# zju3dv/SMAP

Hardware: NVIDIA H100
Metric: end-to-end FPS @832x512 (backbone+association+lift) (higher is better)
Workload: dtype bf16x3 (split-bf16 operands, fp32 accumulate; fp32-faithful)

## Files before the change

smap_b200/csrc/conv_tc.cuh:

```cuda
#pragma once
#include <cuda.h>
#include "common.cuh"

namespace smapb {

struct alignas(64) ConvParams {
    CUtensorMap tmA;
    CUtensorMap tmA2;
    CUtensorMap tmB;
    CUtensorMap tmO;
    CUtensorMap tmR[3];
    int Hout, Wout, Nimg;
    int tw_log2, th;
    int tiles_x, tiles_y;
    int Cout;
    int kh, kw, stride, pad_y, pad_x;
    int kchunks;
    int kchunks2, stride2;
    int n_tiles;
    int total_tiles;
    const float* bias;
    int has_res;
    int n_post;
    __nv_bfloat16* out;
    float* out_f32;
    long long plane_stride;
    int relu;
    int reverse;
    int up_mode, up_Hi, up_Wi, up_pw, up_ph;
    long long* dbg;
    long long* dbg_tl;
    unsigned long long* sat;
};

__device__ __forceinline__ void tma_load_5d(uint32_t dst, const CUtensorMap* map, uint64_t* bar, int c0, int c1,
                                            int c2, int c3, int c4) {
    asm volatile(
        "cp.async.bulk.tensor.5d.shared::cluster.global.tile.mbarrier::complete_tx::bytes [%0], [%1, {%3, %4, %5, %6, "
        "%7}], [%2];" ::"r"(dst),
        "l"(map), "r"(smem_u32(bar)), "r"(c0), "r"(c1), "r"(c2), "r"(c3), "r"(c4)
        : "memory");
}
__device__ __forceinline__ void tma_load_4d(uint32_t dst, const CUtensorMap* map, uint64_t* bar, int c0, int c1,
                                            int c2, int c3) {
    asm volatile(
        "cp.async.bulk.tensor.4d.shared::cluster.global.tile.mbarrier::complete_tx::bytes [%0], [%1, {%3, %4, %5, "
        "%6}], [%2];" ::"r"(dst),
        "l"(map), "r"(smem_u32(bar)), "r"(c0), "r"(c1), "r"(c2), "r"(c3)
        : "memory");
}
__device__ __forceinline__ void tma_prefetch_desc(const CUtensorMap* map) {
    asm volatile("prefetch.tensormap [%0];" ::"l"(map) : "memory");
}
__device__ __forceinline__ void tma_store_5d(const CUtensorMap* map, uint32_t src, int c0, int c1, int c2, int c3,
                                             int c4) {
    asm volatile("cp.async.bulk.tensor.5d.global.shared::cta.tile.bulk_group [%0, {%2, %3, %4, %5, %6}], [%1];" ::"l"(map),
                 "r"(src), "r"(c0), "r"(c1), "r"(c2), "r"(c3), "r"(c4)
                 : "memory");
}
__device__ __forceinline__ void bulk_commit() { asm volatile("cp.async.bulk.commit_group;" ::: "memory"); }
template <int N>
__device__ __forceinline__ void bulk_wait_read() {
    asm volatile("cp.async.bulk.wait_group.read %0;" ::"n"(N) : "memory");
}
__device__ __forceinline__ void bulk_wait_all() { asm volatile("cp.async.bulk.wait_group 0;" ::: "memory"); }
enum { TURN_MAIN = 3, TURN_RING = 5 };
__device__ __forceinline__ void epi_bar_sync(int wg) { asm volatile("bar.sync %0, 128;" ::"r"(1 + wg) : "memory"); }
__device__ __forceinline__ void turn_wait(int turn, int wg) { asm volatile("bar.sync %0, 256;" ::"r"(turn + wg) : "memory"); }
__device__ __forceinline__ void turn_pass(int turn, int wg) { asm volatile("bar.arrive %0, 256;" ::"r"(turn + wg) : "memory"); }
template <int R>
__device__ __forceinline__ void setmaxnreg_dec() {
    asm volatile("setmaxnreg.dec.sync.aligned.u32 %0;" ::"n"(R));
}
template <int R>
__device__ __forceinline__ void setmaxnreg_inc() {
    asm volatile("setmaxnreg.inc.sync.aligned.u32 %0;" ::"n"(R));
}
struct ConvDbg {
    enum {
        PRODUCER_WAIT_EMPTY = 0,
        TOTAL = 1,
        CTAS = 2,
        CONS = 3,
        WAIT_FULL = 0,
        WAIT_ORDER = 1,
        EPILOGUE = 2,
        WAIT_RING = 3,
        WAIT_STAGE = 4,
        CONS_N = 5,
        COUNT = CONS + 2 * CONS_N
    };
};
__device__ __forceinline__ uint32_t lds_u32(uint32_t addr) {
    uint32_t r;
    asm volatile("ld.shared.u32 %0, [%1];" : "=r"(r) : "r"(addr));
    return r;
}
__device__ __forceinline__ void sts_u32(uint32_t addr, uint32_t v) {
    asm volatile("st.shared.u32 [%0], %1;" ::"r"(addr), "r"(v) : "memory");
}
__device__ __forceinline__ uint32_t sw64_off(int r, int j) { return (uint32_t)(r * 64 + ((j ^ ((r >> 1) & 3)) << 4)); }

__device__ __forceinline__ float up_scale(int in, int out) { return out > 1 ? (float)(in - 1) / (float)(out - 1) : 0.f; }
__device__ __forceinline__ int up_src_index(int dst, int in, int out) { return (int)(up_scale(in, out) * (float)dst); }

__device__ __forceinline__ float2 planes_to_f2(uint32_t h, uint32_t l) {
    return make_float2(bf16lo_to_f(h) + bf16lo_to_f(l), bf16hi_to_f(h) + bf16hi_to_f(l));
}

__device__ __forceinline__ uint64_t wgmma_desc_sw128(uint32_t smem_addr) {
    uint64_t d = 0;
    d |= (uint64_t)((smem_addr >> 4) & 0x3FFF);
    d |= (uint64_t)1 << 16;
    d |= (uint64_t)(1024 >> 4) << 32;
    d |= (uint64_t)1 << 62;
    return d;
}
__device__ __forceinline__ void wgmma_fence() { asm volatile("wgmma.fence.sync.aligned;" ::: "memory"); }
__device__ __forceinline__ void wgmma_commit() { asm volatile("wgmma.commit_group.sync.aligned;" ::: "memory"); }
template <int N>
__device__ __forceinline__ void wgmma_wait() {
    asm volatile("wgmma.wait_group.sync.aligned %0;" ::"n"(N) : "memory");
}
template <class E>
__device__ __forceinline__ void wgmma_m64n128(float (&d)[64], uint64_t adesc, uint64_t bdesc, uint32_t accumulate) {
#define SMAPB_WGMMA(TY) \
    asm volatile( \
        "{\n\t.reg .pred p;\n\tsetp.ne.b32 p, %66, 0;\n\t" \
        "wgmma.mma_async.sync.aligned.m64n128k16.f32." TY "." TY " {%0, %1, %2, %3, %4, %5, %6, %7, %8, %9, %10, %11, %12, " \
        "%13, %14, %15, %16, %17, %18, %19, %20, %21, %22, %23, %24, %25, %26, %27, %28, %29, %30, %31, %32, %33, %34, %35, " \
        "%36, %37, %38, %39, %40, %41, %42, %43, %44, %45, %46, %47, %48, %49, %50, %51, %52, %53, %54, %55, %56, %57, %58, " \
        "%59, %60, %61, %62, %63}, %64, %65, p, 1, 1, 0, 0;\n\t}" \
        : "+f"(d[0]), "+f"(d[1]), "+f"(d[2]), "+f"(d[3]), "+f"(d[4]), "+f"(d[5]), "+f"(d[6]), "+f"(d[7]), "+f"(d[8]), \
          "+f"(d[9]), "+f"(d[10]), "+f"(d[11]), "+f"(d[12]), "+f"(d[13]), "+f"(d[14]), "+f"(d[15]), "+f"(d[16]), \
          "+f"(d[17]), "+f"(d[18]), "+f"(d[19]), "+f"(d[20]), "+f"(d[21]), "+f"(d[22]), "+f"(d[23]), "+f"(d[24]), \
          "+f"(d[25]), "+f"(d[26]), "+f"(d[27]), "+f"(d[28]), "+f"(d[29]), "+f"(d[30]), "+f"(d[31]), "+f"(d[32]), \
          "+f"(d[33]), "+f"(d[34]), "+f"(d[35]), "+f"(d[36]), "+f"(d[37]), "+f"(d[38]), "+f"(d[39]), "+f"(d[40]), \
          "+f"(d[41]), "+f"(d[42]), "+f"(d[43]), "+f"(d[44]), "+f"(d[45]), "+f"(d[46]), "+f"(d[47]), "+f"(d[48]), \
          "+f"(d[49]), "+f"(d[50]), "+f"(d[51]), "+f"(d[52]), "+f"(d[53]), "+f"(d[54]), "+f"(d[55]), "+f"(d[56]), \
          "+f"(d[57]), "+f"(d[58]), "+f"(d[59]), "+f"(d[60]), "+f"(d[61]), "+f"(d[62]), "+f"(d[63]) \
        : "l"(adesc), "l"(bdesc), "r"(accumulate))
    if constexpr (E::F16) SMAPB_WGMMA("f16");
    else SMAPB_WGMMA("bf16");
#undef SMAPB_WGMMA
}
template <class E>
__device__ __forceinline__ void wgmma_m64n64(float (&d)[32], uint64_t adesc, uint64_t bdesc, uint32_t accumulate) {
#define SMAPB_WGMMA(TY) \
    asm volatile( \
        "{\n\t.reg .pred p;\n\tsetp.ne.b32 p, %34, 0;\n\t" \
        "wgmma.mma_async.sync.aligned.m64n64k16.f32." TY "." TY " {%0, %1, %2, %3, %4, %5, %6, %7, %8, %9, %10, %11, %12, " \
        "%13, %14, %15, %16, %17, %18, %19, %20, %21, %22, %23, %24, %25, %26, %27, %28, %29, %30, %31}, %32, %33, p, 1, " \
        "1, 0, 0;\n\t}" \
        : "+f"(d[0]), "+f"(d[1]), "+f"(d[2]), "+f"(d[3]), "+f"(d[4]), "+f"(d[5]), "+f"(d[6]), "+f"(d[7]), "+f"(d[8]), \
          "+f"(d[9]), "+f"(d[10]), "+f"(d[11]), "+f"(d[12]), "+f"(d[13]), "+f"(d[14]), "+f"(d[15]), "+f"(d[16]), \
          "+f"(d[17]), "+f"(d[18]), "+f"(d[19]), "+f"(d[20]), "+f"(d[21]), "+f"(d[22]), "+f"(d[23]), "+f"(d[24]), \
          "+f"(d[25]), "+f"(d[26]), "+f"(d[27]), "+f"(d[28]), "+f"(d[29]), "+f"(d[30]), "+f"(d[31]) \
        : "l"(adesc), "l"(bdesc), "r"(accumulate))
    if constexpr (E::F16) SMAPB_WGMMA("f16");
    else SMAPB_WGMMA("bf16");
#undef SMAPB_WGMMA
}
template <class E>
__device__ __forceinline__ void wgmma_m64n32(float (&d)[16], uint64_t adesc, uint64_t bdesc, uint32_t accumulate) {
#define SMAPB_WGMMA(TY) \
    asm volatile( \
        "{\n\t.reg .pred p;\n\tsetp.ne.b32 p, %18, 0;\n\t" \
        "wgmma.mma_async.sync.aligned.m64n32k16.f32." TY "." TY " {%0, %1, %2, %3, %4, %5, %6, %7, %8, %9, %10, %11, %12, " \
        "%13, %14, %15}, %16, %17, p, 1, 1, 0, 0;\n\t}" \
        : "+f"(d[0]), "+f"(d[1]), "+f"(d[2]), "+f"(d[3]), "+f"(d[4]), "+f"(d[5]), "+f"(d[6]), "+f"(d[7]), "+f"(d[8]), \
          "+f"(d[9]), "+f"(d[10]), "+f"(d[11]), "+f"(d[12]), "+f"(d[13]), "+f"(d[14]), "+f"(d[15]) \
        : "l"(adesc), "l"(bdesc), "r"(accumulate))
    if constexpr (E::F16) SMAPB_WGMMA("f16");
    else SMAPB_WGMMA("bf16");
#undef SMAPB_WGMMA
}
template <int BLOCK_N, class E>
__device__ __forceinline__ void wgmma_tile(float (&d)[BLOCK_N / 2], uint64_t adesc, uint64_t bdesc, uint32_t accumulate) {
    if constexpr (BLOCK_N == 128) wgmma_m64n128<E>(d, adesc, bdesc, accumulate);
    else if constexpr (BLOCK_N == 64) wgmma_m64n64<E>(d, adesc, bdesc, accumulate);
    else wgmma_m64n32<E>(d, adesc, bdesc, accumulate);
}

__device__ __forceinline__ long long mbar_wait_timed(uint64_t* bar, uint32_t parity, bool timed) {
    if (!timed) {
        mbar_wait(bar, parity);
        return 0;
    }
    const long long t0 = clock64();
    mbar_wait(bar, parity);
    return clock64() - t0;
}

template <int BLOCK_N, int NTERMS, int RING>
struct ConvCfg {
    static constexpr int TA = (NTERMS == 3) ? 2 : 1;
    static constexpr int A_BYTES = 128 * 128;
    static constexpr int B_BYTES = BLOCK_N * 128;
    static constexpr int STAGE_BYTES = TA * (A_BYTES + B_BYTES);
    static constexpr int CHUNKS = BLOCK_N / 32;
    static constexpr int CHUNK_BYTES = 128 * 64;
    static constexpr int SLOT_BYTES = TA * CHUNK_BYTES;
    static constexpr int RES_BUFS = RING ? 2 : 0;
    static constexpr int RES_DIV = RING ? RES_BUFS : 1;
    static constexpr int SMEM_LIMIT = 227 * 1024;
    static constexpr int stages_with(int out_bufs) {
        return (SMEM_LIMIT - 2048 - (out_bufs + RES_BUFS) * SLOT_BYTES) / STAGE_BYTES > 8
                   ? 8
                   : (SMEM_LIMIT - 2048 - (out_bufs + RES_BUFS) * SLOT_BYTES) / STAGE_BYTES;
    }
    static constexpr int OUT_PER_WG = stages_with(4) == stages_with(2) ? 2 : 1;
    static constexpr int OUT_BUFS = 2 * OUT_PER_WG;
    static constexpr int EPI_BYTES = (OUT_BUFS + RES_BUFS) * SLOT_BYTES;
    static constexpr int STAGES = stages_with(OUT_BUFS);
    static constexpr int SMEM_BYTES = STAGES * STAGE_BYTES + EPI_BYTES + 2048;
    static_assert(STAGES >= 2, "need at least a double buffer");
    static_assert(BLOCK_N == 32 || BLOCK_N == 64 || BLOCK_N == 128, "BLOCK_N");
};

template <int BLOCK_N, int NTERMS, int RING, class E>
__global__ void __launch_bounds__(384, 1) conv_tc_kernel(const __grid_constant__ ConvParams p) {
    static_assert(!E::F16 || NTERMS == 1, "fp16 operands are single-term");
    using Cfg = ConvCfg<BLOCK_N, NTERMS, RING>;
    constexpr int STAGES = Cfg::STAGES;
    constexpr bool UP = (RING == 2);
    extern __shared__ unsigned char smem_raw[];
    uint64_t* full_bar = reinterpret_cast<uint64_t*>(smem_raw);
    uint64_t* empty_bar = full_bar + STAGES;
    uint64_t* rfull_bar = empty_bar + STAGES;
    uint64_t* rempty_bar = rfull_bar + Cfg::RES_BUFS;
    const uint32_t ring = (smem_u32(smem_raw) + 1024u + 1023u) & ~1023u;
    const uint32_t out_stage = ring + STAGES * Cfg::STAGE_BYTES;
    const uint32_t res_stage = out_stage + Cfg::OUT_BUFS * Cfg::SLOT_BYTES;

    const int warp = threadIdx.x >> 5;
    const int lane = threadIdx.x & 31;
    const bool tl = p.dbg_tl != nullptr && blockIdx.x == 0;
    if (tl && threadIdx.x == 0) p.dbg_tl[0] = clock64();
    const int n_extra = RING ? p.has_res + p.n_post : 0;
    const bool tma_out = p.out != nullptr;

    if (warp == 0 && lane == 0) {
        tma_prefetch_desc(&p.tmA);
        tma_prefetch_desc(&p.tmB);
        if (p.kchunks2) tma_prefetch_desc(&p.tmA2);
        if (tma_out) tma_prefetch_desc(&p.tmO);
        for (int e = 0; e < n_extra; e++) tma_prefetch_desc(&p.tmR[e]);
    }
    if (warp == 1 && lane == 0) {
        for (int s = 0; s < STAGES; s++) {
            mbar_init(&full_bar[s], 1);
            mbar_init(&empty_bar[s], 4);
        }
        for (int s = 0; s < Cfg::RES_BUFS; s++) {
            mbar_init(&rfull_bar[s], 1);
            mbar_init(&rempty_bar[s], 128);
        }
        fence_mbar_init();
    }
    __syncthreads();

    const int num_kb1 = p.kh * p.kw * p.kchunks;
    const int num_kb = num_kb1 + p.kchunks2;
    const int tiles_per_img = p.tiles_x * p.tiles_y;
    const int tw = 1 << p.tw_log2;

    if (tl && threadIdx.x == 0) p.dbg_tl[1] = clock64();
    pdl_wait();
    pdl_trigger();
    const long long t_begin = p.dbg ? clock64() : 0;

    if (warp < 4) {
        setmaxnreg_dec<40>();
        if (warp == 0 && lane == 0) {
            int stage = 0;
            uint32_t phase = 0;
            long long w_empty = 0;
            for (int tile = blockIdx.x; tile < p.total_tiles; tile += gridDim.x) {
                const int te = p.reverse ? p.total_tiles - 1 - tile : tile;
                const int nt = te % p.n_tiles, mt = te / p.n_tiles;
                const int img = mt / tiles_per_img, r = mt - img * tiles_per_img;
                const int ty = r / p.tiles_x, tx = r - ty * p.tiles_x;
                const int x_in0 = (tx << p.tw_log2) * p.stride - p.pad_x;
                const int y_in0 = ty * p.th * p.stride - p.pad_y;
                for (int kb = 0; kb < num_kb; kb++) {
                    w_empty += mbar_wait_timed(&empty_bar[stage], phase ^ 1u, p.dbg != nullptr);
                    const uint32_t sbase = ring + stage * Cfg::STAGE_BYTES;
                    mbar_arrive_expect_tx(&full_bar[stage], Cfg::STAGE_BYTES);
                    const int brow = nt * BLOCK_N;
                    int kcol, tapc, ax, ay;
                    const CUtensorMap* amap;
                    if (kb < num_kb1) {
                        const int ts = kb / p.kchunks, kc = kb - ts * p.kchunks;
                        const int kx = ts / p.kh, ky = ts - kx * p.kh;
                        amap = &p.tmA, kcol = kc * 64, tapc = ky * p.kw + kx, ax = x_in0 + kx, ay = y_in0 + ky;
                    } else {
                        const int kc2 = kb - num_kb1;
                        amap = &p.tmA2, kcol = kc2 * 64, tapc = 0;
                        ax = (tx << p.tw_log2) * p.stride2, ay = ty * p.th * p.stride2;
                    }
                    const int wcol = (kb < num_kb1) ? kcol : (p.kchunks * 64 + kcol);
#pragma unroll
                    for (int t = 0; t < Cfg::TA; t++) {
                        const uint32_t da = sbase + t * Cfg::A_BYTES, db = sbase + Cfg::TA * Cfg::A_BYTES + t * Cfg::B_BYTES;
                        tma_load_5d(da, amap, &full_bar[stage], kcol, ax, ay, img, t);
                        tma_load_4d(db, &p.tmB, &full_bar[stage], wcol, brow, tapc, t);
                    }
                    if (++stage == STAGES) {
                        stage = 0;
                        phase ^= 1u;
                    }
                }
            }
            if (p.dbg) atomicAdd((unsigned long long*)&p.dbg[ConvDbg::PRODUCER_WAIT_EMPTY], (unsigned long long)w_empty);
        } else if (warp == 1 && lane == 0 && n_extra > 0) {
            int cnt = 0;
            for (int tile = blockIdx.x; tile < p.total_tiles; tile += gridDim.x) {
                const int te = p.reverse ? p.total_tiles - 1 - tile : tile;
                const int nt = te % p.n_tiles, mt = te / p.n_tiles;
                const int img = mt / tiles_per_img, r = mt - img * tiles_per_img;
                const int ty = r / p.tiles_x, tx = r - ty * p.tiles_x;
                for (int c = 0; c < Cfg::CHUNKS; c++) {
                    for (int e = 0; e < n_extra; e++) {
                        const int m = cnt++;
                        const int slot = m % Cfg::RES_DIV;
                        mbar_wait(&rempty_bar[slot], ((uint32_t)(m / Cfg::RES_DIV) & 1u) ^ 1u);
                        int cx = tx << p.tw_log2, cy = ty * p.th;
                        uint32_t bytes = Cfg::SLOT_BYTES;
                        if (UP && e == 0) {
                            cx = up_src_index(cx, p.up_Wi, p.Wout);
                            cy = up_src_index(cy, p.up_Hi, p.Hout);
                            bytes = (uint32_t)(p.up_pw * p.up_ph * 64 * Cfg::TA);
                        }
                        mbar_arrive_expect_tx(&rfull_bar[slot], bytes);
#pragma unroll
                        for (int t = 0; t < Cfg::TA; t++)
                            tma_load_5d(res_stage + slot * Cfg::SLOT_BYTES + t * Cfg::CHUNK_BYTES, &p.tmR[e],
                                        &rfull_bar[slot], nt * BLOCK_N + c * 32, cx, cy, img, t);
                    }
                }
            }
        }
    } else {
        setmaxnreg_inc<232>();
        const int wg = (warp >> 2) - 1;
        const int q4 = lane & 3;
        const int rw = (warp & 3) * 16 + (lane >> 2);
        const bool leader = (threadIdx.x & 127) == 0;
        const bool timed = p.dbg != nullptr && leader;
        const uint32_t ob0 = out_stage + (uint32_t)(wg * Cfg::OUT_PER_WG) * Cfg::SLOT_BYTES;
        const int n_cta = (p.total_tiles - (int)blockIdx.x + (int)gridDim.x - 1) / (int)gridDim.x;
        long long* const dc = p.dbg ? p.dbg + ConvDbg::CONS + ConvDbg::CONS_N * wg : nullptr;
        auto tally = [&](int k, long long cycles) {
            if (timed) atomicAdd((unsigned long long*)&dc[k], (unsigned long long)cycles);
        };
        float acc[2][BLOCK_N / 2];
        for (int j = wg; j < n_cta; j += 2) {
            const int tile = blockIdx.x + j * gridDim.x;
            const int te = p.reverse ? p.total_tiles - 1 - tile : tile;
            const int nt = te % p.n_tiles, mt = te / p.n_tiles;
            const int img = mt / tiles_per_img, r = mt - img * tiles_per_img;
            const int ty = r / p.tiles_x, tx = r - ty * p.tiles_x;
            const int n0 = nt * BLOCK_N;

            const uint32_t it0 = (uint32_t)j * (uint32_t)num_kb;
            int stage = (int)(it0 % STAGES);
            uint32_t phase = (it0 / STAGES) & 1u;
            if (j > 0) {
                const long long t0 = timed ? clock64() : 0;
                turn_wait(TURN_MAIN, wg);
                tally(ConvDbg::WAIT_ORDER, timed ? clock64() - t0 : 0);
            }
            int prev_stage = -1;
            uint32_t w_full = 0;
            for (int kb = 0; kb < num_kb; kb++) {
                w_full += (uint32_t)mbar_wait_timed(&full_bar[stage], phase, timed);
                if (tl && leader && j == 0 && kb == 0) p.dbg_tl[2] = clock64();
                const uint32_t sbase = ring + stage * Cfg::STAGE_BYTES;
                const uint64_t a0 = wgmma_desc_sw128(sbase);
                const uint64_t b0 = wgmma_desc_sw128(sbase + Cfg::TA * Cfg::A_BYTES);
                constexpr uint64_t A_STEP = (uint64_t)(Cfg::A_BYTES >> 4), B_STEP = (uint64_t)(Cfg::B_BYTES >> 4);
                constexpr uint64_t A_HALF = (uint64_t)((64 * 128) >> 4);
                wgmma_fence();
#pragma unroll
                for (int k = 0; k < 4; k++) {
#pragma unroll
                    for (int h = 0; h < 2; h++) {
                        const uint64_t ka = a0 + (uint64_t)(k * 2) + h * A_HALF, kbd = b0 + (uint64_t)(k * 2);
                        wgmma_tile<BLOCK_N, E>(acc[h], ka, kbd, (kb | k) != 0);
                        if (NTERMS == 3) {
                            wgmma_tile<BLOCK_N, E>(acc[h], ka + A_STEP, kbd, 1u);
                            wgmma_tile<BLOCK_N, E>(acc[h], ka, kbd + B_STEP, 1u);
                        }
                    }
                }
                wgmma_commit();
                wgmma_wait<1>();
                if (prev_stage >= 0 && lane == 0) mbar_arrive(&empty_bar[prev_stage]);
                prev_stage = stage;
                if (++stage == STAGES) {
                    stage = 0;
                    phase ^= 1u;
                }
            }
            if (j + 1 < n_cta) turn_pass(TURN_MAIN, wg ^ 1);
            tally(ConvDbg::WAIT_FULL, w_full);
            wgmma_wait<0>();
            if (lane == 0) mbar_arrive(&empty_bar[prev_stage]);
            if (tl && leader && j == n_cta - 1) p.dbg_tl[3] = clock64();

            const long long t_epi0 = timed ? clock64() : 0;
            int py[4], px[4];
            bool valid[4];
            long long pix[4];
#pragma unroll
            for (int q = 0; q < 4; q++) {
                const int row = 64 * (q >> 1) + rw + 8 * (q & 1);
                py[q] = ty * p.th + (row >> p.tw_log2);
                px[q] = (tx << p.tw_log2) + (row & (tw - 1));
                valid[q] = (py[q] < p.Hout) && (px[q] < p.Wout) && (img < p.Nimg);
                pix[q] = ((long long)img * p.Hout + py[q]) * p.Wout + px[q];
            }
            auto row_of = [&](int q) { return 64 * (q >> 1) + rw + 8 * (q & 1); };
            const bool ring_turns = RING != 0 && n_extra > 0;
            if (ring_turns && j > 0) turn_wait(TURN_RING, wg);
            int rcnt = j * Cfg::CHUNKS * n_extra;
            auto ring_wait = [&]() -> uint32_t {
                const int m = rcnt++;
                const int rslot = m % Cfg::RES_DIV;
                tally(ConvDbg::WAIT_RING, mbar_wait_timed(&rfull_bar[rslot], (uint32_t)(m / Cfg::RES_DIV) & 1u, timed));
                return (uint32_t)rslot;
            };
            auto ring_release = [&](uint32_t rslot) {
                fence_proxy_async();
                mbar_arrive(&rempty_bar[rslot]);
            };
            auto ring_f2 = [&](uint32_t rb, uint32_t o) -> float2 {
                if constexpr (E::F16) {
                    const uint32_t w = lds_u32(rb + o);
                    return make_float2(E::lo(w), E::hi(w));
                } else {
                    return planes_to_f2(lds_u32(rb + o), NTERMS == 3 ? lds_u32(rb + Cfg::CHUNK_BYTES + o) : 0u);
                }
            };
            auto ring_add = [&](float(&vv)[4][8]) {
                const uint32_t rslot = ring_wait();
                const uint32_t rb = res_stage + rslot * Cfg::SLOT_BYTES;
#pragma unroll
                for (int q = 0; q < 4; q++)
#pragma unroll
                    for (int jj = 0; jj < 4; jj++) {
                        const uint32_t o = sw64_off(row_of(q), jj) + 4 * q4;
                        const float2 rv = ring_f2(rb, o);
                        vv[q][2 * jj] += rv.x;
                        vv[q][2 * jj + 1] += rv.y;
                    }
                ring_release(rslot);
            };
#pragma unroll
            for (int c = 0; c < Cfg::CHUNKS; c++) {
                const int c0 = c * 32;
                float v[4][8];
#pragma unroll
                for (int jj = 0; jj < 4; jj++) {
                    const float2 bia = __ldg(reinterpret_cast<const float2*>(p.bias + n0 + c0 + 8 * jj + 2 * q4));
                    const int f = 4 * (4 * c + jj);
#pragma unroll
                    for (int h = 0; h < 2; h++) {
                        v[2 * h][2 * jj] = acc[h][f + 0] + bia.x;
                        v[2 * h][2 * jj + 1] = acc[h][f + 1] + bia.y;
                        v[2 * h + 1][2 * jj] = acc[h][f + 2] + bia.x;
                        v[2 * h + 1][2 * jj + 1] = acc[h][f + 3] + bia.y;
                    }
                }
                if (RING == 1 && p.has_res) ring_add(v);
                if (UP) {
                    const uint32_t rslot = ring_wait();
                    const uint32_t rb = res_stage + rslot * Cfg::SLOT_BYTES;
                    const int oy0 = up_src_index(ty * p.th, p.up_Hi, p.Hout), ox0 = up_src_index(tx << p.tw_log2, p.up_Wi, p.Wout);
#pragma unroll
                    for (int q = 0; q < 4; q++) {
                        const int pyc = min(py[q], p.Hout - 1), pxc = min(px[q], p.Wout - 1);
                        const float sy = up_scale(p.up_Hi, p.Hout) * (float)pyc, sx = up_scale(p.up_Wi, p.Wout) * (float)pxc;
                        const int y0i = (int)sy, x0i = (int)sx;
                        const int y1i = y0i + (y0i < p.up_Hi - 1 ? 1 : 0), x1i = x0i + (x0i < p.up_Wi - 1 ? 1 : 0);
                        const float hy1 = sy - (float)y0i, hy0 = 1.f - hy1, wx1 = sx - (float)x0i, wx0 = 1.f - wx1;
                        const int rr[4] = {(y0i - oy0) * p.up_pw + (x0i - ox0), (y0i - oy0) * p.up_pw + (x1i - ox0),
                                           (y1i - oy0) * p.up_pw + (x0i - ox0), (y1i - oy0) * p.up_pw + (x1i - ox0)};
#pragma unroll
                        for (int jj = 0; jj < 4; jj++) {
                            float2 s[4];
#pragma unroll
                            for (int k = 0; k < 4; k++) {
                                const uint32_t o = sw64_off(rr[k], jj) + 4 * q4;
                                s[k] = ring_f2(rb, o);
                            }
                            v[q][2 * jj] += hy0 * (wx0 * s[0].x + wx1 * s[1].x) + hy1 * (wx0 * s[2].x + wx1 * s[3].x);
                            v[q][2 * jj + 1] += hy0 * (wx0 * s[0].y + wx1 * s[1].y) + hy1 * (wx0 * s[2].y + wx1 * s[3].y);
                        }
                    }
                    ring_release(rslot);
                }
                if (p.relu) {
#pragma unroll
                    for (int q = 0; q < 4; q++)
#pragma unroll
                        for (int e = 0; e < 8; e++) v[q][e] = fmaxf(v[q][e], 0.f);
                }
                for (int e = 0; RING == 1 && e < p.n_post; e++) ring_add(v);
                if (tma_out) {
                    const uint32_t ob = ob0 + (uint32_t)((((j >> 1) * Cfg::CHUNKS + c) % Cfg::OUT_PER_WG) * Cfg::SLOT_BYTES);
                    if (leader) {
                        const long long t0 = timed ? clock64() : 0;
                        bulk_wait_read<Cfg::OUT_PER_WG - 1>();
                        tally(ConvDbg::WAIT_STAGE, timed ? clock64() - t0 : 0);
                    }
                    bool sat_warp = false;
                    if constexpr (E::F16) {
                        float m = 0.f;
#pragma unroll
                        for (int q = 0; q < 4; q++)
#pragma unroll
                            for (int e = 0; e < 8; e++) m = E::absmax(m, v[q][e]);
                        sat_warp = __any_sync(0xffffffffu, !(m <= E::MAX));
                    }
                    epi_bar_sync(wg);
                    int n_sat = 0;
#pragma unroll
                    for (int q = 0; q < 4; q++)
#pragma unroll
                        for (int jj = 0; jj < 4; jj++) {
                            const float a = v[q][2 * jj], b = v[q][2 * jj + 1];
                            const uint32_t o = sw64_off(row_of(q), jj) + 4 * q4;
                            if constexpr (E::F16) {
                                if (sat_warp) {
                                    int n = 0;
                                    sts_u32(ob + o, E::pack2(E::clamp(a, n), E::clamp(b, n)));
                                    n_sat += valid[q] ? n : 0;
                                } else {
                                    sts_u32(ob + o, E::pack2(a, b));
                                }
                            } else {
                                const uint32_t hw = E::pack2(a, b);
                                sts_u32(ob + o, hw);
                                if (NTERMS == 3)
                                    sts_u32(ob + Cfg::CHUNK_BYTES + o, E::pack2(a - E::lo(hw), b - E::hi(hw)));
                            }
                        }
                    if constexpr (E::F16)
                        if (sat_warp) saturation_add(p.sat, n_sat);
                    fence_proxy_async();
                    epi_bar_sync(wg);
                    if (leader) {
#pragma unroll
                        for (int t = 0; t < Cfg::TA; t++)
                            tma_store_5d(&p.tmO, ob + t * Cfg::CHUNK_BYTES, n0 + c0, tx << p.tw_log2, ty * p.th, img, t);
                        bulk_commit();
                    }
                } else {
#pragma unroll
                    for (int q = 0; q < 4; q++) {
                        if (!valid[q]) continue;
#pragma unroll
                        for (int jj = 0; jj < 4; jj++)
                            *reinterpret_cast<float2*>(p.out_f32 + pix[q] * p.Cout + n0 + c0 + 8 * jj + 2 * q4) =
                                make_float2(v[q][2 * jj], v[q][2 * jj + 1]);
                    }
                }
            }
            if (ring_turns && j + 1 < n_cta) turn_pass(TURN_RING, wg ^ 1);
            tally(ConvDbg::EPILOGUE, timed ? clock64() - t_epi0 : 0);
        }
        if (leader && tma_out) bulk_wait_all();
        if (leader && wg == ((n_cta - 1) & 1)) {
            if (p.dbg) {
                atomicAdd((unsigned long long*)&p.dbg[ConvDbg::TOTAL], (unsigned long long)(clock64() - t_begin));
                atomicAdd((unsigned long long*)&p.dbg[ConvDbg::CTAS], 1ull);
            }
            if (tl) p.dbg_tl[13] = p.dbg_tl[15] = clock64();
        }
    }
}

}
```

Measured before the change: 481.6.

## Load A-hi fragments via ldmatrix and issue register-sourced WGMMA for bf16x3 terms

For the three-term split-bf16 path, the high part of A is loaded into registers with ldmatrix and reused by two register-sourced WGMMAs per k-step, while the low-A term stays shared-memory sourced. The single commit per k-block becomes one commit per k-slice, with a wait<1> and an earlier release of the previous stage. Epilogue pixel coordinates are recomputed on demand instead of held in arrays, to reduce register pressure from the extra fragment registers. The aim is to cut shared-memory operand reads, at the cost of more commit/wait points and a proxy fence before each stage release.

```diff
diff --git a/smap_b200/csrc/conv_tc.cuh b/smap_b200/csrc/conv_tc.cuh
--- a/smap_b200/csrc/conv_tc.cuh
+++ b/smap_b200/csrc/conv_tc.cuh
@@ -181,6 +181,61 @@
     else if constexpr (BLOCK_N == 64) wgmma_m64n64<E>(d, adesc, bdesc, accumulate);
     else wgmma_m64n32<E>(d, adesc, bdesc, accumulate);
 }
+__device__ __forceinline__ void wgmma_rs_m64n128(float (&d)[64], const uint32_t (&a)[4], uint64_t bdesc, uint32_t accumulate) {
+    asm volatile(
+        "{\n\t.reg .pred p;\n\tsetp.ne.b32 p, %69, 0;\n\t"
+        "wgmma.mma_async.sync.aligned.m64n128k16.f32.bf16.bf16 {%0, %1, %2, %3, %4, %5, %6, %7, %8, %9, %10, %11, %12, "
+        "%13, %14, %15, %16, %17, %18, %19, %20, %21, %22, %23, %24, %25, %26, %27, %28, %29, %30, %31, %32, %33, %34, %35, "
+        "%36, %37, %38, %39, %40, %41, %42, %43, %44, %45, %46, %47, %48, %49, %50, %51, %52, %53, %54, %55, %56, %57, %58, "
+        "%59, %60, %61, %62, %63}, {%64, %65, %66, %67}, %68, p, 1, 1, 0;\n\t}"
+        : "+f"(d[0]), "+f"(d[1]), "+f"(d[2]), "+f"(d[3]), "+f"(d[4]), "+f"(d[5]), "+f"(d[6]), "+f"(d[7]), "+f"(d[8]),
+          "+f"(d[9]), "+f"(d[10]), "+f"(d[11]), "+f"(d[12]), "+f"(d[13]), "+f"(d[14]), "+f"(d[15]), "+f"(d[16]),
+          "+f"(d[17]), "+f"(d[18]), "+f"(d[19]), "+f"(d[20]), "+f"(d[21]), "+f"(d[22]), "+f"(d[23]), "+f"(d[24]),
+          "+f"(d[25]), "+f"(d[26]), "+f"(d[27]), "+f"(d[28]), "+f"(d[29]), "+f"(d[30]), "+f"(d[31]), "+f"(d[32]),
+          "+f"(d[33]), "+f"(d[34]), "+f"(d[35]), "+f"(d[36]), "+f"(d[37]), "+f"(d[38]), "+f"(d[39]), "+f"(d[40]),
+          "+f"(d[41]), "+f"(d[42]), "+f"(d[43]), "+f"(d[44]), "+f"(d[45]), "+f"(d[46]), "+f"(d[47]), "+f"(d[48]),
+          "+f"(d[49]), "+f"(d[50]), "+f"(d[51]), "+f"(d[52]), "+f"(d[53]), "+f"(d[54]), "+f"(d[55]), "+f"(d[56]),
+          "+f"(d[57]), "+f"(d[58]), "+f"(d[59]), "+f"(d[60]), "+f"(d[61]), "+f"(d[62]), "+f"(d[63])
+        : "r"(a[0]), "r"(a[1]), "r"(a[2]), "r"(a[3]), "l"(bdesc), "r"(accumulate));
+}
+__device__ __forceinline__ void wgmma_rs_m64n64(float (&d)[32], const uint32_t (&a)[4], uint64_t bdesc, uint32_t accumulate) {
+    asm volatile(
+        "{\n\t.reg .pred p;\n\tsetp.ne.b32 p, %37, 0;\n\t"
+        "wgmma.mma_async.sync.aligned.m64n64k16.f32.bf16.bf16 {%0, %1, %2, %3, %4, %5, %6, %7, %8, %9, %10, %11, %12, "
+        "%13, %14, %15, %16, %17, %18, %19, %20, %21, %22, %23, %24, %25, %26, %27, %28, %29, %30, %31}, "
+        "{%32, %33, %34, %35}, %36, p, 1, 1, 0;\n\t}"
+        : "+f"(d[0]), "+f"(d[1]), "+f"(d[2]), "+f"(d[3]), "+f"(d[4]), "+f"(d[5]), "+f"(d[6]), "+f"(d[7]), "+f"(d[8]),
+          "+f"(d[9]), "+f"(d[10]), "+f"(d[11]), "+f"(d[12]), "+f"(d[13]), "+f"(d[14]), "+f"(d[15]), "+f"(d[16]),
+          "+f"(d[17]), "+f"(d[18]), "+f"(d[19]), "+f"(d[20]), "+f"(d[21]), "+f"(d[22]), "+f"(d[23]), "+f"(d[24]),
+          "+f"(d[25]), "+f"(d[26]), "+f"(d[27]), "+f"(d[28]), "+f"(d[29]), "+f"(d[30]), "+f"(d[31])
+        : "r"(a[0]), "r"(a[1]), "r"(a[2]), "r"(a[3]), "l"(bdesc), "r"(accumulate));
+}
+__device__ __forceinline__ void wgmma_rs_m64n32(float (&d)[16], const uint32_t (&a)[4], uint64_t bdesc, uint32_t accumulate) {
+    asm volatile(
+        "{\n\t.reg .pred p;\n\tsetp.ne.b32 p, %21, 0;\n\t"
+        "wgmma.mma_async.sync.aligned.m64n32k16.f32.bf16.bf16 {%0, %1, %2, %3, %4, %5, %6, %7, %8, %9, %10, %11, %12, "
+        "%13, %14, %15}, {%16, %17, %18, %19}, %20, p, 1, 1, 0;\n\t}"
+        : "+f"(d[0]), "+f"(d[1]), "+f"(d[2]), "+f"(d[3]), "+f"(d[4]), "+f"(d[5]), "+f"(d[6]), "+f"(d[7]), "+f"(d[8]),
+          "+f"(d[9]), "+f"(d[10]), "+f"(d[11]), "+f"(d[12]), "+f"(d[13]), "+f"(d[14]), "+f"(d[15])
+        : "r"(a[0]), "r"(a[1]), "r"(a[2]), "r"(a[3]), "l"(bdesc), "r"(accumulate));
+}
+template <int BLOCK_N>
+__device__ __forceinline__ void wgmma_tile_rs(float (&d)[BLOCK_N / 2], const uint32_t (&a)[4], uint64_t bdesc,
+                                              uint32_t accumulate) {
+    if constexpr (BLOCK_N == 128) wgmma_rs_m64n128(d, a, bdesc, accumulate);
+    else if constexpr (BLOCK_N == 64) wgmma_rs_m64n64(d, a, bdesc, accumulate);
+    else wgmma_rs_m64n32(d, a, bdesc, accumulate);
+}
+__device__ __forceinline__ void ldsm_a_sw128(uint32_t (&a)[4], uint32_t tile, int row0, int k) {
+    const int l = threadIdx.x & 31;
+    const uint32_t lane0 = (uint32_t)((16 * ((threadIdx.x >> 5) & 3) + (l & 7) + 8 * ((l >> 3) & 1)) * 128) +
+                           (uint32_t)(((l >> 4) ^ (l & 7)) << 4);
+    const uint32_t addr = ((tile + lane0) ^ (uint32_t)(k << 5)) + (uint32_t)(row0 * 128);
+    asm volatile("ldmatrix.sync.aligned.m8n8.x4.shared.b16 {%0, %1, %2, %3}, [%4];"
+                 : "=r"(a[0]), "=r"(a[1]), "=r"(a[2]), "=r"(a[3])
+                 : "r"(addr)
+                 : "memory");
+}
 
 __device__ __forceinline__ long long mbar_wait_timed(uint64_t* bar, uint32_t parity, bool timed) {
     if (!timed) {
@@ -371,8 +426,17 @@
                 turn_wait(TURN_MAIN, wg);
                 tally(ConvDbg::WAIT_ORDER, timed ? clock64() - t0 : 0);
             }
+            constexpr bool RS = (NTERMS == 3);
+            auto release = [&](int s) {
+                if constexpr (RS) {
+                    fence_proxy_async();
+                    __syncwarp();
+                }
+                if (lane == 0) mbar_arrive(&empty_bar[s]);
+            };
             int prev_stage = -1;
             uint32_t w_full = 0;
+            uint32_t fa[2][2][4];
             for (int kb = 0; kb < num_kb; kb++) {
                 w_full += (uint32_t)mbar_wait_timed(&full_bar[stage], phase, timed);
                 if (tl && leader && j == 0 && kb == 0) p.dbg_tl[2] = clock64();
@@ -381,22 +445,36 @@
                 const uint64_t b0 = wgmma_desc_sw128(sbase + Cfg::TA * Cfg::A_BYTES);
                 constexpr uint64_t A_STEP = (uint64_t)(Cfg::A_BYTES >> 4), B_STEP = (uint64_t)(Cfg::B_BYTES >> 4);
                 constexpr uint64_t A_HALF = (uint64_t)((64 * 128) >> 4);
-                wgmma_fence();
-#pragma unroll
-                for (int k = 0; k < 4; k++) {
-#pragma unroll
-                    for (int h = 0; h < 2; h++) {
-                        const uint64_t ka = a0 + (uint64_t)(k * 2) + h * A_HALF, kbd = b0 + (uint64_t)(k * 2);
-                        wgmma_tile<BLOCK_N, E>(acc[h], ka, kbd, (kb | k) != 0);
-                        if (NTERMS == 3) {
+                if constexpr (RS) {
+#pragma unroll
+                    for (int k = 0; k < 4; k++) {
+                        uint32_t(&f)[2][4] = fa[k & 1];
+                        wgmma_wait<1>();
+                        if (k == 1 && prev_stage >= 0) release(prev_stage);
+#pragma unroll
+                        for (int h = 0; h < 2; h++) ldsm_a_sw128(f[h], sbase, 64 * h, k);
+                        wgmma_fence();
+#pragma unroll
+                        for (int h = 0; h < 2; h++) {
+                            const uint64_t ka = a0 + (uint64_t)(k * 2) + h * A_HALF, kbd = b0 + (uint64_t)(k * 2);
+                            wgmma_tile_rs<BLOCK_N>(acc[h], f[h], kbd, (kb | k) != 0);
                             wgmma_tile<BLOCK_N, E>(acc[h], ka + A_STEP, kbd, 1u);
-                            wgmma_tile<BLOCK_N, E>(acc[h], ka, kbd + B_STEP, 1u);
+                            wgmma_tile_rs<BLOCK_N>(acc[h], f[h], kbd + B_STEP, 1u);
                         }
-                    }
-                }
-                wgmma_commit();
-                wgmma_wait<1>();
-                if (prev_stage >= 0 && lane == 0) mbar_arrive(&empty_bar[prev_stage]);
+                        wgmma_commit();
+                    }
+                } else {
+                    wgmma_fence();
+#pragma unroll
+                    for (int k = 0; k < 4; k++)
+#pragma unroll
+                        for (int h = 0; h < 2; h++)
+                            wgmma_tile<BLOCK_N, E>(acc[h], a0 + (uint64_t)(k * 2) + h * A_HALF, b0 + (uint64_t)(k * 2),
+                                                   (kb | k) != 0);
+                    wgmma_commit();
+                    wgmma_wait<1>();
+                    if (prev_stage >= 0) release(prev_stage);
+                }
                 prev_stage = stage;
                 if (++stage == STAGES) {
                     stage = 0;
@@ -406,22 +484,14 @@
             if (j + 1 < n_cta) turn_pass(TURN_MAIN, wg ^ 1);
             tally(ConvDbg::WAIT_FULL, w_full);
             wgmma_wait<0>();
-            if (lane == 0) mbar_arrive(&empty_bar[prev_stage]);
+            release(prev_stage);
             if (tl && leader && j == n_cta - 1) p.dbg_tl[3] = clock64();
 
             const long long t_epi0 = timed ? clock64() : 0;
-            int py[4], px[4];
-            bool valid[4];
-            long long pix[4];
-#pragma unroll
-            for (int q = 0; q < 4; q++) {
-                const int row = 64 * (q >> 1) + rw + 8 * (q & 1);
-                py[q] = ty * p.th + (row >> p.tw_log2);
-                px[q] = (tx << p.tw_log2) + (row & (tw - 1));
-                valid[q] = (py[q] < p.Hout) && (px[q] < p.Wout) && (img < p.Nimg);
-                pix[q] = ((long long)img * p.Hout + py[q]) * p.Wout + px[q];
-            }
             auto row_of = [&](int q) { return 64 * (q >> 1) + rw + 8 * (q & 1); };
+            auto py_of = [&](int q) { return ty * p.th + (row_of(q) >> p.tw_log2); };
+            auto px_of = [&](int q) { return (tx << p.tw_log2) + (row_of(q) & (tw - 1)); };
+            auto valid_of = [&](int q) { return (py_of(q) < p.Hout) && (px_of(q) < p.Wout) && (img < p.Nimg); };
             const bool ring_turns = RING != 0 && n_extra > 0;
             if (ring_turns && j > 0) turn_wait(TURN_RING, wg);
             int rcnt = j * Cfg::CHUNKS * n_extra;
@@ -480,7 +550,7 @@
                     const int oy0 = up_src_index(ty * p.th, p.up_Hi, p.Hout), ox0 = up_src_index(tx << p.tw_log2, p.up_Wi, p.Wout);
 #pragma unroll
                     for (int q = 0; q < 4; q++) {
-                        const int pyc = min(py[q], p.Hout - 1), pxc = min(px[q], p.Wout - 1);
+                        const int pyc = min(py_of(q), p.Hout - 1), pxc = min(px_of(q), p.Wout - 1);
                         const float sy = up_scale(p.up_Hi, p.Hout) * (float)pyc, sx = up_scale(p.up_Wi, p.Wout) * (float)pxc;
                         const int y0i = (int)sy, x0i = (int)sx;
                         const int y1i = y0i + (y0i < p.up_Hi - 1 ? 1 : 0), x1i = x0i + (x0i < p.up_Wi - 1 ? 1 : 0);
@@ -536,7 +606,7 @@
                                 if (sat_warp) {
                                     int n = 0;
                                     sts_u32(ob + o, E::pack2(E::clamp(a, n), E::clamp(b, n)));
-                                    n_sat += valid[q] ? n : 0;
+                                    n_sat += valid_of(q) ? n : 0;
                                 } else {
                                     sts_u32(ob + o, E::pack2(a, b));
                                 }
@@ -560,10 +630,11 @@
                 } else {
 #pragma unroll
                     for (int q = 0; q < 4; q++) {
-                        if (!valid[q]) continue;
+                        if (!valid_of(q)) continue;
+                        const long long pix = ((long long)img * p.Hout + py_of(q)) * p.Wout + px_of(q);
 #pragma unroll
                         for (int jj = 0; jj < 4; jj++)
-                            *reinterpret_cast<float2*>(p.out_f32 + pix[q] * p.Cout + n0 + c0 + 8 * jj + 2 * q4) =
+                            *reinterpret_cast<float2*>(p.out_f32 + pix * p.Cout + n0 + c0 + 8 * jj + 2 * q4) =
                                 make_float2(v[q][2 * jj], v[q][2 * jj + 1]);
                     }
                 }
```

Result: faster. 490.3, median of 6 (+1.8%).
